# VatsalSy/gerris-fft-particles

Measured on AMD Instinct MI355X. Metric: Mcell-steps/s (projection+advection), 3D 256^3 uniform, higher is better.
Workload: dtype f64; 1 GPU; 3-D periodic Taylor-Green, 256^3 per GPU, default projection/advection parameters (SURVEY 8d config C); relax_mode=exact, parallelism=1 box, rccl_world_size=0

## Files before the change

### gerris-fft-particles_amd/csrc/gfship_internal.hpp

```cpp
#pragma once

#include <hip/hip_runtime.h>
#include <cstdio>
#include <cstdarg>
#include <cstring>
#include <vector>
#include <deque>
#include <string>
#include "gfship.h"

namespace gfship {

struct Layout {
  int n = 0;
  int px = 0;
  int xo = 1;
  int rows = 0;
  int dim = 3;
  long sy = 0;
  long sz = 0;
  size_t total = 0;
  __host__ __device__ inline long idx (int i, int j, int k) const {
    return xo + i + sy*j + sz*k;
  }
// ... 126 lines not shown
    if (e_ != hipSuccess) return gfship::hip_fail (e_, #call, __FILE__, __LINE__); } while (0)

inline hipError_t stream_wait_spin (hipStream_t st)
{
  hipError_t e;
  while ((e = hipStreamQuery (st)) == hipErrorNotReady)
    ;
  return e;
}

#define GFSHIP_CHECK(cond, code, ...) do { if (!(cond)) { \
    gfship::set_error (__VA_ARGS__); return (code); } } while (0)

Field * get_field (gfship_domain * dom, gfship_field f);
int coarse_flush (gfship_domain * dom, Field * F, int level, bool leaf_write = false);
inline long ncells (const Layout & L) {
  return L.dim == 3 ? (long) L.n*L.n*L.n : (long) L.n*L.n;
}

int launch_bc (gfship_domain * dom, Field * v, Field * v1, int level, int homogeneous);
int call_exchange (gfship_domain * dom, double * ptr, int level, int kind);
int bc_mpi_begin (gfship_domain * dom, Field * v1, int level);
int bc_mpi_end (gfship_domain * dom, Field * v, Field * v1, int level, int homogeneous);
int call_reduce (gfship_domain * dom, double * vals, int n, int op);
int call_reduce_norm (gfship_domain * dom, double * sums, int nsum, double * mx);
int comm_exchange (gfship_domain * dom, double * a, int level, int kind);
int comm_exchange_raw (gfship_domain * dom, double * const send[6], double * const recv[6], size_t count);
int comm_migrate (gfship_domain * dom, int rs, const int nsend[6], const double * const send[6],
		  int nrecv[6], std::vector<double> recv[6]);
int comm_allgather (gfship_domain * dom, const double * send, double * recv, size_t count);
// ... 27 lines not shown
int launch_residual (gfship_domain * dom, int level, const double * u, const double * rhs,
		     const double * dia, double * res);
int launch_residual_weighted (gfship_domain * dom, int level, const double * u, const double * rhs,
			      const double * dia, double * res);
int launch_poisson_weights (gfship_domain * dom, double * const alpha[3]);
RelaxOp weighted_op (gfship_domain * dom, int level);
int launch_restrict (gfship_domain * dom, unsigned dimension, int level_coarse, double * v_coarse,
		     const double * v_fine);
int launch_prolongate (gfship_domain * dom, int level_coarse, const double * v_coarse,
		       double * v_fine);
int launch_correct (gfship_domain * dom, int level, double * u, const double * dp);
int launch_fill (gfship_domain * dom, int level, double * a, double value);
int launch_residual_norm (gfship_domain * dom, int level, const double * u, const double * rhs,
			  const double * dia, double * res, double scale, double weight,
			  double * out , bool dia_zero = false);
int launch_norm_async (gfship_domain * dom, int level, const double * a, double scale, double weight);
int launch_norm (gfship_domain * dom, int level, const double * a, double scale, double weight,
		 double out[5] );

int launch_face_interp_un (gfship_domain * dom, double * const u[3], double * const un[3]);
int launch_divergence (gfship_domain * dom, double * const un[3], double * div, double dt);
int launch_correct_un (gfship_domain * dom, const double * p, double * const un[3], double dt);
int launch_centered_gradient (gfship_domain * dom, const double * p, double * const g[3]);
int launch_correct_centered (gfship_domain * dom, double * const u[3], double * const g[3], double dt);
int launch_correct_centered_coarse (gfship_domain * dom, double * const u[3], double * const g[3],
				    double dt, double * const uc[3]);
int launch_coarse_init_from (gfship_domain * dom, Field * const * v, int nf, int top);
int launch_coarse_init_levels (gfship_domain * dom, Field * const * v, int nf, int top, int bottom);
int launch_advected_face_values (gfship_domain * dom, const double * v, double * const u[3],
				 double * const un[3], double dt, int use_centered, int gradient,
				 double * const fv[6], int cmask, double visc = 0., double gsrc = 0.);
// ... 43 lines not shown
		     const double * dia, bool dia_zero, unsigned nrelax, int reps,
		     double * ms_per_loop, int * fused, double * ms_inclusive = nullptr);
int  skew_check_error (gfship_domain * dom);
int  skew_arm_ahead (gfship_domain * dom, int level, unsigned nrelax);
int  patch_resident_per_cu ();
bool prolongation_fused (gfship_domain * dom, unsigned dimension, int level, unsigned nrelax);
bool prolongation_fusable (gfship_domain * dom, unsigned dimension, int level, unsigned nrelax);
inline bool patch_level (const gfship_domain * dom, int level) { return dom->patch && !dom->weighted && dom->lay[level].n >= dom->patch_min_n; }
int  patch_pack (gfship_domain * dom, int level, SkewPlan * S, const double * u, const double * rhs,
		 const double * dia, const double * coarse = nullptr);
int  patch_unpack (gfship_domain * dom, int level, SkewPlan * S, double * u, double * add_into);
int  patch_restrict_pack (gfship_domain * dom, int level, SkewPlan * S, const double * res,
			  double * res_coarse, SkewPlan * Sc, unsigned dimension);
int  launch_restrict_pack (gfship_domain * dom, unsigned dimension, int level, Field * res,
			   bool coarse_fused);
void skew_dump_stats (gfship_domain * dom, int level);
int  skew_time_sweeps (gfship_domain * dom, int level, Field * u, const double * rhs,
		       const double * dia, bool dia_zero, int reps, double * ms_per_sweep);

}
```

### gerris-fft-particles_amd/csrc/poisson.hip

```cpp
#include "gfship_internal.hpp"
#include <cmath>
#include <cfloat>
#include <cstdlib>

using namespace gfship;

namespace gfship {

static bool weighted_pipelinable (gfship_domain * dom, unsigned dimension, int level)
{
  return dom->relax_mode == GFSHIP_RELAX_EXACT && dimension == 3 && dom->dim == 3 &&
    skew_supported (dom, level) && !dom->force_hyperplane;
}

static bool weighted_pipelined (gfship_domain * dom, unsigned dimension, int level)
{
  static const bool off = getenv ("GFSHIP_WEIGHTED_HYPERPLANES") != nullptr;
  return !off && weighted_pipelinable (dom, dimension, level);
}

static int relax_level (gfship_domain * dom, unsigned dimension, int level, double omega,
			Field * u, Field * rhs, Field * dia)
{
  u->zero[level] = false;
// ... 282 lines not shown
  if (n.w > 0.) {
    n.bias /= n.w;
    n.first /= n.w;
    n.second = sqrt (n.second/n.w);
  }
  else
    n.infty = 0.;
  *out = n;
  return GFSHIP_OK;
}

}

static int poisson_cycle (gfship_domain * dom, gfship_multilevel_params * p,
			  gfship_field u, gfship_field rhs, gfship_field dia, gfship_field res,
			  double dt, gfship_norm * norm)
{
  GFSHIP_CHECK (dom && p, GFSHIP_EINVAL, "null argument");
  GFSHIP_CHECK (p->dimension == 2 || p->dimension == 3, GFSHIP_EINVAL, "dimension must be 2 or 3");
  GFSHIP_CHECK (p->nrelax > 0 && p->erelax > 0, GFSHIP_EINVAL, "nrelax and erelax must be non zero");
  GFSHIP_CHECK (dom->unit_weights, GFSHIP_EINVAL, "call gfship_poisson_coefficients first");
  if (dom->dp_cache < 0)
    dom->dp_cache = gfship_field_alloc (dom, -1);
  gfship_field dpf = dom->dp_cache;
  if (dpf < 0) return dpf;
  Field * U = get_field (dom, u), * R = get_field (dom, rhs), * D = get_field (dom, dia),
    * S = get_field (dom, res), * DP = get_field (dom, dpf);
  int r = GFSHIP_OK;
  bool corrected = false;
  if (!U || !R || !D || !S) return GFSHIP_EINVAL;
  const int L = dom->depth;
// ... 9 lines not shown
    {
      unsigned nr = p->nrelax;
      for (int l = L; l >= 0; l--) {
	nrl[l] = nr;
	if (l > (int) minlevel) nr *= p->erelax;
      }
    }
    for (int l = 0; l <= L; l++)
      DP->zero[l] = false;
    const int ctop = dom->weighted ? -1 : coarse_cycle_top (dom, (int) minlevel);
    const int ltop = ctop >= 0 ? -1 : lattice_cycle_top (dom, (int) minlevel, D);
    for (int l = L - 1; l >= (ctop >= 0 ? ctop + 1 : ltop >= 0 ? ltop : 0); l--) {
      if (dom->relax_mode == GFSHIP_RELAX_EXACT && p->dimension == 3 && !dom->weighted &&
	  !dom->force_hyperplane && skew_supported (dom, l + 1))
	TRY (skew_arm_ahead (dom, l + 1, nrl[l + 1]));
      const bool rp = !dom->skew[l + 1].rs_ready && prolongation_fused (dom, p->dimension, l + 1, nrl[l + 1]);
      if (rp) dom->kc[dom->no_fused_restriction ? GFSHIP_KC_RESTRICTION_DECLINED : GFSHIP_KC_RESTRICTION_FUSED]++;
      if (!dom->no_fused_restriction && rp)
	TRY (launch_restrict_pack (dom, p->dimension, l + 1, S,
				   l > (int) minlevel && prolongation_fused (dom, p->dimension, l, nrl[l])));
      else
	TRY (launch_restrict (dom, p->dimension, l, S->lev[l], S->lev[l + 1]));
    }
    unsigned first = minlevel;
    if (ltop >= 0) {
      TRY (launch_lattice_cycle (dom, p->dimension, p->omega, (int) minlevel, ltop, nrl, DP, U, S));
      first = ltop + 1;
    }
    else if (ctop >= 0) {
      TRY (launch_coarse_cycle (dom, p->dimension, p->omega, (int) minlevel, ctop, nrl, DP, U, S, D));
// ... 5 lines not shown
      first = minlevel + 1;
      dom->kc[GFSHIP_KC_COARSE_END_BY_LEVEL]++;
    }
    for (unsigned l = first; l <= p->depth; l++) {
      const bool fp = prolongation_fused (dom, p->dimension, (int) l, nrl[l]);
      if (fp) dom->kc[GFSHIP_KC_PROLONGATION_FUSED]++;
      else if (prolongation_fusable (dom, p->dimension, (int) l, nrl[l])) dom->kc[GFSHIP_KC_PROLONGATION_DECLINED]++;
      if (!fp)
	TRY (launch_prolongate (dom, l - 1, DP->lev[l - 1], DP->lev[l]));
      TRY (relax_loop (dom, DP, U, p->dimension, l, p->omega, S, D, nrl[l],
		       (int) l == L ? U->lev[L] : nullptr, &corrected, fp ? DP->lev[l - 1] : nullptr));
    }
  }
  if (!corrected)
    TRY (launch_correct (dom, L, U->lev[L], DP->lev[L]));
  TRY (launch_bc (dom, U, U, L, 0));
  if (norm)
    TRY (residual_and_norm (dom, dt, U, R, D, S, norm));
  else if (dom->weighted)
    TRY (launch_residual_weighted (dom, L, U->lev[L], R->lev[L], D->lev[L], S->lev[L]));
  else
    TRY (launch_residual (dom, L, U->lev[L], R->lev[L], D->lev[L], S->lev[L]));
#undef TRY
 done:
  for (int l = 0; l <= L; l++)
    dom->skew[l].rs_ready = false;
  return r;
}

extern "C" {

int gfship_poisson_cycle (gfship_domain * dom, gfship_multilevel_params * p,
			  gfship_field u, gfship_field rhs, gfship_field dia, gfship_field res)
{
  GFSHIP_CHECK (dom != nullptr, GFSHIP_EINVAL, "null domain");
  int r = before_write (dom);
  if (r) return r;
  return poisson_cycle (dom, p, u, rhs, dia, res, 1., nullptr);
}

int gfship_poisson_solve (gfship_domain * dom, gfship_multilevel_params * par,
			  gfship_field lhs, gfship_field rhs, gfship_field res,
// ... 1 lines not shown
{
  GFSHIP_CHECK (dom && par, GFSHIP_EINVAL, "null argument");
  Field * U = get_field (dom, lhs), * R = get_field (dom, rhs), * D = get_field (dom, dia),
    * S = get_field (dom, res);
  if (!U || !R || !D || !S) return GFSHIP_EINVAL;
  GFSHIP_CHECK (dom->unit_weights, GFSHIP_EINVAL, "call gfship_poisson_coefficients first");
  { int r = before_write (dom); if (r) return r; }
  int r;
  const int L = dom->depth;
  if ((r = coarse_flush (dom, U, L, true))) return r;
  unsigned minlevel = par->minlevel;
  par->depth = L;
  par->niter = 0;

  bool deferred = par->nitermin >= 1 && par->nitermax >= 1;
  if (deferred) {
    const Layout & Ly = dom->lay[L];
    double size = 1./Ly.n;
    S->zero[L] = false;
    if (dom->weighted) {
      if ((r = launch_residual_weighted (dom, L, U->lev[L], R->lev[L], D->lev[L], S->lev[L]))) return r;
      if ((r = launch_norm_async (dom, L, S->lev[L], 1.*size*size, 1.))) return r;
    }
    else if ((r = launch_residual_norm (dom, L, U->lev[L], R->lev[L], D->lev[L], S->lev[L], 1.*size*size,
					1., nullptr, D->zero[L])))
      return r;
  }
  else {
    if ((r = residual_and_norm (dom, dt, U, R, D, S, &par->residual))) return r;
    par->residual_before = par->residual;
  }

  double res_max_before = par->residual.infty;

  while (par->niter < par->nitermin ||
	 (par->residual.infty > par->tolerance && par->niter < par->nitermax)) {
    if ((r = poisson_cycle (dom, par, lhs, rhs, dia, res, dt, &par->residual))) {
      if (deferred) {
	deferred = false;
	double s0[5];
	if (hipStreamSynchronize (dom->stream) == hipSuccess) {
	  memcpy (s0, dom->h_pinned + 8, sizeof (s0));
	  if (norm_residual_finish (dom, dt, s0, &par->residual_before) == GFSHIP_OK)
	    par->residual = par->residual_before;
	}
	else
	  memset (&par->residual_before, 0, sizeof (par->residual_before)),
	    memset (&par->residual, 0, sizeof (par->residual));
      }
      break;
    }
    if (deferred) {
// ... 80 lines not shown
```

### gerris-fft-particles_amd/csrc/poisson_kernels.hip

```cpp
#include "gfship_internal.hpp"
#include "relax_skew.hpp"
#include <algorithm>
#include <cstdlib>

namespace gfship {

struct W6 { const double * p[6]; };

template <int DIM, int OP>
__device__ __forceinline__ double relax_value (const double * __restrict__ u, long c, long sy, long sz,
					       double rhs, double dia, unsigned dimension,
					       double omega, double w, double h2, const W6 * wf = nullptr)
{
  if (OP == 2) {
    double a = dia, b = 0.;
    { const double g = wf->p[0][c]; a += g; b += g*u[c + 1]; }
    { const double g = wf->p[1][c]; a += g; b += g*u[c - 1]; }
    { const double g = wf->p[2][c]; a += g; b += g*u[c + sy]; }
    { const double g = wf->p[3][c]; a += g; b += g*u[c - sy]; }
    if (DIM == 3) {
      { const double g = wf->p[4][c]; a += g; b += g*u[c + sz]; }
      { const double g = wf->p[5][c]; a += g; b += g*u[c - sz]; }
    }
    if (dimension == 2)
// ... 1515 lines not shown
int launch_norm_async (gfship_domain * dom, int level, const double * a, double scale, double weight)
{
  const Layout & L = dom->lay[level];
  long nrows = L.dim == 3 ? (long) L.n*L.n : L.n;
  int block = L.n >= 256 ? 256 : L.n >= 128 ? 128 : 64;
  int nblocks = (int) (nrows > 1024 ? 1024 : nrows);
  double * partial = dom->d_scratch;
  double * result = dom->h_pinned + 8;
  NORM_PARTIAL_LAUNCH ();
  hipLaunchKernelGGL (norm_final_kernel, dim3 (1), dim3 (256), 0, dom->stream,
		      partial, nblocks, result);
  GFSHIP_HIP (hipGetLastError ());
  return GFSHIP_OK;
}

int launch_norm (gfship_domain * dom, int level, const double * a, double scale, double weight,
		 double out[5])
{
  const Layout & L = dom->lay[level];
  long nrows = L.dim == 3 ? (long) L.n*L.n : L.n;
  int block = L.n >= 256 ? 256 : L.n >= 128 ? 128 : 64;
  int nblocks = (int) (nrows > 1024 ? 1024 : nrows);
  double * partial = dom->d_scratch;
  double * result = dom->h_pinned;
  NORM_PARTIAL_LAUNCH ();
  hipLaunchKernelGGL (norm_final_kernel, dim3 (1), dim3 (256), 0, dom->stream,
		      partial, nblocks, result);
  GFSHIP_HIP (hipGetLastError ());
  GFSHIP_HIP (stream_wait_spin (dom->stream));
  memcpy (out, dom->h_pinned, 5*sizeof (double));
// ... 112 lines not shown
  s0 = wave_sum (s0); s1 = wave_sum (s1); s2 = wave_sum (s2); s3 = wave_max (s3); s4 = wave_sum (s4);
  int w = threadIdx.x >> 6, lane = threadIdx.x & 63;
  if (lane == 0) { sh[0][w] = s0; sh[1][w] = s1; sh[2][w] = s2; sh[3][w] = s3; sh[4][w] = s4; }
  __syncthreads ();
  if (threadIdx.x == 0) {
    int nw = blockDim.x >> 6;
    double r0 = 0., r1 = 0., r2 = 0., r3 = 0., r4 = 0.;
    for (int q = 0; q < nw; q++) {
      r0 += sh[0][q]; r1 += sh[1][q]; r2 += sh[2][q]; r3 = fmax (r3, sh[3][q]); r4 += sh[4][q];
    }
    double * p = partial + 5*(size_t) blockIdx.x;
    p[0] = r0; p[1] = r1; p[2] = r2; p[3] = r3; p[4] = r4;
  }
}

int launch_residual_norm (gfship_domain * dom, int level, const double * u, const double * rhs,
			  const double * dia, double * res, double scale, double weight,
			  double * out, bool dia_zero)
{
  const Layout & L = dom->lay[level];
  if (!power_of_two (scale)) {
    int r = launch_residual (dom, level, u, rhs, dia, res);
    if (r) return r;
    return out ? launch_norm (dom, level, res, scale, weight, out) :
      launch_norm_async (dom, level, res, scale, weight);
  }
  long nrows = L.dim == 3 ? (long) L.n*L.n : L.n;
  int block = L.n >= 256 ? 256 : L.n >= 128 ? 128 : 64;
  static int rn_blocks = 0;
  if (!rn_blocks) {
// ... 192 lines not shown
```

### gerris-fft-particles_amd/csrc/relax_patch_loop.hip

```cpp
#include "relax_skew.hpp"
#include <cstdlib>
#include <vector>

#ifndef PK_D
#define PK_D 9
#endif
#ifndef PK_DH
#define PK_DH 3
#endif
#ifndef PK_KO
#define PK_KO 0
#endif
#define PK_NTHREADS 192
#define PK_SKEW 14

namespace gfship {

typedef double d2 __attribute__((ext_vector_type(2)));

__device__ __forceinline__ void patch_arm_other_set (const SkewLoopArgs & A, int tile, int tid, int nt)
{
  if (A.arm_pairs == 0) return;
  typedef unsigned long long ull2 __attribute__((ext_vector_type(2)));
  const unsigned long long W = A.arm_cum[A.ntj*A.ntj];
// ... 827 lines not shown
  }
  const double v = __longlong_as_double ((long long) bits);
  A.un[dst] = sg == 0. ? v : sg*v;
}

struct PatchPackArgs {
  Layout L;
  int ntj, RT;
  const double * src[3];
  double * dst[3];
  int narr;
  double * add;
  const double * coarse;
  double * nat;
  Layout Lc;
};

__device__ __forceinline__ double patch_prolong (const Layout & Lc, const double * __restrict__ vc,
						 int i, int j, int k)
{
  const int pi = (i + 1)/2, pj = (j + 1)/2, pk = (k + 1)/2;
  const long p = Lc.idx (pi, pj, pk);
  const double pv = vc[p];
  double h[3];
  const long off[3] = { 1, Lc.sy, Lc.sz };
#pragma unroll
  for (int cc = 0; cc < 3; cc++) {
    double g1 = vc[p + off[cc]] - 1.*pv;
    double g2 = vc[p - off[cc]] - 1.*pv;
    h[cc] = (g1 - g2)/2.;
  }
// ... 100 lines not shown
    const double bx = pv + ((I & 1) ? qx : - qx);
    d2 o01, o23;
    {
      const double by0 = bx + qy, by1 = bx + (- qy);
      o01.x = by0 + qz;     o01.y = by1 + qz;
      o23.x = by0 + (- qz); o23.y = by1 + (- qz);
    }
    double * const row = dst + (long) rho*SK_NL;
    *(d2 *) row = o01;
    *(d2 *) (row + 128) = o23;
    if (__builtin_expect (I == 0 || I == n - 1 || side_j[0] || side_j[1] || side_k[0] || side_k[1], 0)) {
      const bool ends = I == 0 || I == n - 1;
      const double vv[4] = { o01.x, o01.y, o23.x, o23.y };
#pragma unroll
      for (int q = 0; q < 4; q++)
	if (ends || side_j[q & 1] || side_k[q >> 1])
	  A.nat[A.L.idx (I + 1, j0 - (q & 1), k0 - (q >> 1))] = vv[q];
    }
  }
}

#ifndef PP_ROWS
#define PP_ROWS 16
#endif
#define PP_SPAN (PP_ROWS + 7)
#ifndef PPR_ROWS
#define PPR_ROWS 64
#endif
#define PPR_SPAN (PPR_ROWS + 7)
#ifndef PPU_ROWS
#define PPU_ROWS 64
#endif
// ... 8 lines not shown
  const int P = tile % A.ntj, Q = tile / A.ntj;
  const int n = A.L.n;
  const long tbase = (long) tile*(A.RT + 2*SK_FP)*SK_NL + SK_FP*SK_NL;
  const int I0 = r0 - 7 - PB;
  for (int e = tid; e < 32*PP_SPAN; e += 256) {
    const int line = e / PP_SPAN, di = e % PP_SPAN;
    const int a = line & 15, db = line >> 4;
    const int I = I0 + di;
    if (I >= 0 && I < n) {
      const int j = n - (SK_T*P + a), k = n - (SK_T*Q + 2*PB + db);
      const long nidx = A.L.idx (I + 1, j, k);
      int q0 = 0;
      if (A.coarse) {
	const double v = patch_prolong (A.Lc, A.coarse, I + 1, j, k);
	buf[0][line][di] = v;
	if (I == 0 || I == n - 1 || j == 1 || j == n || k == 1 || k == n)
	  A.nat[nidx] = v;
	q0 = 1;
      }
      for (int q = q0; q < A.narr; q++)
	buf[q][line][di] = A.src[q][nidx];
    }
  }
  __syncthreads ();
  for (int e = tid; e < PP_ROWS*32; e += 256) {
    const int row = e / 32, col = e % 32;
    const int PA = col >> 2, p = col & 3;
    const int a = 2*PA + (p & 1), db = p >> 1;
    const int rho = r0 + row;
    const int I = rho - PA - PB;
    if (I >= 0 && I < n) {
      const long sidx = tbase + (long) rho*SK_NL + 128*(p >> 1) + 2*(PA + 8*PB) + (p & 1);
// ... 53 lines not shown
      double val = 0.;
#pragma unroll
      for (int id = 0; id < 8; id++)
	val += buf[2*PA + ((id >> 1) & 1) + 16*(id >> 2)][di + (id & 1)];
      const double v = A.dimension == 2 ? val : val/2.;
      const int m = I >> 1;
      const int pj = (n - SK_T*P - 2*PA) >> 1, pk = (n - SK_T*Q - 2*PB) >> 1;
      A.cnat[A.Lc.idx (m + 1, pj, pk)] = v;
      if (A.cskew) {
	const int ca = 8*(P & 1) + PA, cb = 8*(Q & 1) + PB;
	const long ctile = (P >> 1) + (long) A.cntj*(Q >> 1);
	A.cskew[ctile*(A.cRT + 2*SK_FP)*SK_NL + SK_FP*SK_NL +
		(long) (m + (ca >> 1) + (cb >> 1))*SK_NL + 128*(cb & 1) + 2*((ca >> 1) + 8*(cb >> 1)) + (ca & 1)] = v;
      }
    }
  }
}

__global__ void __launch_bounds__(256)
patch_unpack_kernel (PatchPackArgs A)
{
  __shared__ double buf[32][PPU_SPAN + 1];
  const int tid = threadIdx.x;
  const int tile = blockIdx.z, PB = blockIdx.y, r0 = blockIdx.x*PPU_ROWS;
  const int P = tile % A.ntj, Q = tile / A.ntj;
  const int n = A.L.n;
  const long tbase = (long) tile*(A.RT + 2*SK_FP)*SK_NL + SK_FP*SK_NL;
  const int I0 = r0 - 7 - PB;
  for (int e = tid; e < PPU_ROWS*32; e += 256) {
    const int row = e / 32, col = e % 32;
// ... 1 lines not shown
    const int a = 2*PA + (p & 1), db = p >> 1;
    const int rho = r0 + row;
    const int I = rho - PA - PB;
    if (I >= 0 && I < n)
      buf[a + 16*db][I - I0] = A.src[0][tbase + (long) rho*SK_NL + 128*(p >> 1) + 2*(PA + 8*PB) + (p & 1)];
  }
  __syncthreads ();
  for (int e = tid; e < 32*PPU_SPAN; e += 256) {
    const int line = e / PPU_SPAN, di = e % PPU_SPAN;
    const int a = line & 15, db = line >> 4;
    const int I = I0 + di;
    const int rho = I + (a >> 1) + PB;
    if (I >= 0 && I < n && rho >= r0 && rho < r0 + PPU_ROWS) {
      const int j = n - (SK_T*P + a), k = n - (SK_T*Q + 2*PB + db);
      const long c = A.L.idx (I + 1, j, k);
      if (A.add)
	A.add[c] += buf[line][di];
      else
	A.dst[0][c] = buf[line][di];
    }
  }
}

static bool patch_regs ()
{
  return getenv ("GFSHIP_PATCH_REGS") != nullptr;
}

int patch_resident_per_cu ()
{
  int per_cu = 0;
  hipError_t e = patch_regs () ?
    hipOccupancyMaxActiveBlocksPerMultiprocessor (&per_cu, relax_patch_loop_kernel<true>, PK_NTHREADS, 0) :
    hipOccupancyMaxActiveBlocksPerMultiprocessor (&per_cu, relax_ring_loop_kernel<true, 0>, RK_NTHREADS, 0);
  int per_cu1 = 0;
  if (e == hipSuccess)
    e = hipOccupancyMaxActiveBlocksPerMultiprocessor (&per_cu1, relax_ring_loop_kernel<true, 1>, RK_NTHREADS, 0);
  if (per_cu1 < per_cu) per_cu = per_cu1;
  return e == hipSuccess ? per_cu : 0;
}

int patch_pack (gfship_domain * dom, int level, SkewPlan * S, const double * u, const double * rhs,
		const double * dia, const double * coarse)
{
  PatchPackArgs A;
  A.add = nullptr;
  A.coarse = coarse;
  A.nat = const_cast<double *> (u);
  A.Lc = dom->lay[level > 0 ? level - 1 : 0];
  A.L = dom->lay[level]; A.ntj = S->ntj; A.RT = S->RT;
  A.narr = 0;
  A.src[A.narr] = u;   A.dst[A.narr++] = S->us;
  if (rhs) { A.src[A.narr] = rhs; A.dst[A.narr++] = S->rs; }
  if (dia) { A.src[A.narr] = dia; A.dst[A.narr++] = S->ds; }
  const int rows = A.L.n + PK_SKEW + 1;
  const bool old_pack = coarse && getenv ("GFSHIP_OLD_PROLONG_PACK");
  if (coarse) dom->kc[old_pack ? GFSHIP_KC_PROLONG_PACK_OLD : GFSHIP_KC_PROLONG_PACK_NEW]++;
  if (coarse && !old_pack) {
    PatchPackArgs Pr = A;
    Pr.narr = 1;
    dim3 pgrid ((rows + PR_ROWS*PR_WAVES - 1)/(PR_ROWS*PR_WAVES), S->ntj*S->ntj);
    hipLaunchKernelGGL (patch_prolong_kernel, pgrid, dim3 (64*PR_WAVES), 0, dom->stream, Pr);
// ... 16 lines not shown
  PatchRestrictArgs A;
  A.L = dom->lay[level]; A.Lc = dom->lay[level - 1];
  A.ntj = S->ntj; A.RT = S->RT;
  A.src = res; A.dst = S->rs;
  A.cnat = res_coarse;
  A.cskew = Sc ? Sc->rs : nullptr;
  A.cntj = Sc ? Sc->ntj : 0; A.cRT = Sc ? Sc->RT : 0;
  A.dimension = dimension;
  const int rows = A.L.n + PK_SKEW + 1;
  dim3 grid ((rows + PPR_ROWS - 1)/PPR_ROWS, 8, S->ntj*S->ntj);
  hipLaunchKernelGGL (patch_restrict_pack_kernel, grid, dim3 (256), 0, dom->stream, A);
  GFSHIP_HIP (hipGetLastError ());
  return GFSHIP_OK;
}

int patch_unpack (gfship_domain * dom, int level, SkewPlan * S, double * u, double * add_into)
{
  PatchPackArgs A;
  A.coarse = nullptr; A.nat = nullptr; A.Lc = dom->lay[level];
  A.L = dom->lay[level]; A.ntj = S->ntj; A.RT = S->RT;
  A.narr = 1;
  A.src[0] = S->us; A.dst[0] = u; A.add = add_into;
  const int rows = A.L.n + PK_SKEW + 1;
  dim3 grid ((rows + PPU_ROWS - 1)/PPU_ROWS, 8, S->ntj*S->ntj);
  hipLaunchKernelGGL (patch_unpack_kernel, grid, dim3 (256), 0, dom->stream, A);
  GFSHIP_HIP (hipGetLastError ());
  return GFSHIP_OK;
}

int patch_loop_launch (gfship_domain * dom, const SkewLoopArgs & A, int ntiles, bool has_dia,
		       unsigned nrelax, float * ms)
{
  if (ms) GFSHIP_HIP (hipEventRecord (dom->ev0, dom->stream));
  if (A.op == 1)
    hipLaunchKernelGGL ((relax_ring_loop_kernel<true, 1>), dim3 (ntiles), dim3 (RK_NTHREADS), 0, dom->stream, A);
  else if (patch_regs ()) {
    if (has_dia)
// ... 26 lines not shown
```

### gerris-fft-particles_amd/csrc/relax_skew.hip

```cpp
#include "relax_skew.hpp"
#include <cstdlib>

namespace gfship {

template <bool HAS_DIA>
__global__ void __launch_bounds__(SK_NL)
relax_skew_kernel (SkewArgs A)
{
  constexpr int XS = SK_T + 1;
  __shared__ double X[2][XS*XS];
  __shared__ double Y[2][XS*XS];
  __shared__ unsigned s_tile;

  const int tid = threadIdx.x;
  const int a = tid & (SK_T - 1), b = tid >> 4;
  const int n = A.L.n;
  const int ntj = A.ntj;
  const long tstride = (long) (A.RT + 2*SK_FP)*SK_NL;
  const long hstride = (long) SK_HROWS (n)*SK_T;

  if (tid == 0)
    s_tile = A.order[atomicAdd (A.ticket, 1u)];
  __syncthreads ();
  const int tile = s_tile;
// ... 450 lines not shown
  SkewPlan * S;
  int r;
  if ((r = skew_plan (dom, level, &S))) return r;
  double * u = dp->lev[level];
  if ((r = skew_loop_trial (dom, level, S, nrelax, bc))) return r;
  if (op && op->kind == 2) {
    if ((r = skew_pack_weights (dom, level, S, op))) return r;
    dia_zero = false;
  }
  const bool fusedp = prolong_from != nullptr && bc && patch_level (dom, level);
  const double * rhs_pack = S->rs_ready && patch_level (dom, level) ? nullptr : rhs;
  S->rs_ready = false;
  if (prolong_from && !fusedp)
    if ((r = launch_prolongate (dom, level - 1, prolong_from, u))) return r;
  if (fusedp && (r = skew_pack (dom, level, S, u, rhs_pack, dia_zero ? nullptr : dia, prolong_from))) return r;
  if (bc && (r = launch_bc (dom, ubc, dp, level, 1))) return r;
  if (!fusedp && (r = skew_pack (dom, level, S, u, rhs_pack, dia_zero ? nullptr : dia))) return r;
  if (!dom->no_fused_loop && skew_loop_supported (dom, level, nrelax, bc)) {
    if ((r = skew_loop_run (dom, level, S, u, !dia_zero, nrelax, nullptr, ubc, op))) return r;
    return skew_unpack (dom, level, S, u, correct_into);
  }
  for (unsigned q = 0; q < nrelax; q++) {
    if ((r = skew_sweep (dom, level, S, u, !dia_zero, op))) return r;
    if (bc && q + 1 < nrelax && (r = launch_bc (dom, ubc, dp, level, 1))) return r;
  }
  return skew_unpack (dom, level, S, u, correct_into);
}

int launch_restrict_pack (gfship_domain * dom, unsigned dimension, int level, Field * res, bool coarse_fused)
{
  SkewPlan * S, * Sc = nullptr;
  int r;
  if ((r = skew_plan (dom, level, &S))) return r;
  if ((r = skew_loop_trial (dom, level, S, 4, true))) return r;
  if (coarse_fused) {
    if ((r = skew_plan (dom, level - 1, &Sc))) return r;
    if ((r = skew_loop_trial (dom, level - 1, Sc, 4, true))) return r;
  }
  res->zero[level - 1] = false;
  if ((r = patch_restrict_pack (dom, level, S, res->lev[level], res->lev[level - 1], Sc, dimension))) return r;
  S->rs_ready = true;
  if (Sc) Sc->rs_ready = true;
  return GFSHIP_OK;
}

void skew_dump_stats (gfship_domain * dom, int level)
{
  SkewPlan & S = dom->skew[level];
  if (!S.stats) return;
  (void) hipStreamSynchronize (dom->stream);
  int nt = S.ntj*S.ntj;
  std::vector<u64> h (4*nt);
  (void) hipMemcpy (h.data (), S.stats, h.size ()*sizeof (u64), hipMemcpyDeviceToHost);
  u64 t0 = ~0ull;
  for (int q = 0; q < nt; q++) if (h[4*q] < t0) t0 = h[4*q];
  for (int Q = 0; Q < S.ntj; Q++)
    for (int P = 0; P < S.ntj; P++) {
      int q = P + S.ntj*Q;
// ... 139 lines not shown
```

### gerris-fft-particles_amd/gfship/__init__.py

```python
import ctypes as C
import os
import sys

import numpy as np

_PKG = os.path.dirname(os.path.dirname(os.path.abspath(__file__)))
LIB_PATH = os.environ.get("GFSHIP_LIB", os.path.join(_PKG, "lib", "libgfship.so"))

SIDE_PERIODIC, SIDE_BOUNDARY, SIDE_EXTERNAL = 0, 1, 2
BC_SYMMETRY, BC_DIRICHLET, BC_NEUMANN = 0, 1, 2
RELAX_EXACT, RELAX_REDBLACK, RELAX_EXACT_HYPERPLANE, RELAX_EXACT_PER_SWEEP = 0, 1, 2, 3


class GfshipError(RuntimeError):
    pass


class Norm(C.Structure):
    _fields_ = [("bias", C.c_double), ("first", C.c_double), ("second", C.c_double),
                ("infty", C.c_double), ("w", C.c_double)]


class MultilevelParams(C.Structure):
    _fields_ = [("tolerance", C.c_double), ("nrelax", C.c_uint), ("erelax", C.c_uint),
# ... 159 lines not shown

UNIQUE_ID_BYTES = 128

KERNEL_COUNT_NAMES = (
    "PREDICT_SWEEP", "PREDICT_SWEEP_MPI", "PREDICT_TILED", "PREDICT_TILED_MPI", "PREDICT_GENERAL",
    "ADVECT3_SWEEP2", "ADVECT3_SWEEP2_MPI", "ADVECT3_SWEEP1", "ADVECT3_TILED", "ADVECT3_TILED_MPI",
    "ADVECT1_TILED_VELOCITY", "ADVECT1_TILED_TRACER", "ADVECT_GENERAL", "CORRECTION_FUSED",
    "CORRECTION_DECLINED", "DIVERGENCE_FUSED", "DIVERGENCE_DECLINED", "DIVERGENCE_SEPARATE",
    "PROJECT_PAIRS", "PROJECT_SCALAR", "RESIDUAL_PAIRS", "RESIDUAL_SCALAR", "RN_BLOCKS_LIMIT",
    "RN_BLOCKS_MAX", "ROWS2D", "HYPERPLANES_2D", "DIFFUSION_PIPELINED", "DIFFUSION_HYPERPLANES",
    "WEIGHTED_PIPELINED", "WEIGHTED_HYPERPLANES", "PROLONGATION_FUSED", "PROLONGATION_DECLINED",
    "RESTRICTION_FUSED", "RESTRICTION_DECLINED", "PROLONG_PACK_NEW", "PROLONG_PACK_OLD",
    "ARM_AHEAD", "ARM_AHEAD_DECLINED", "ARM_INLINE", "PATCH_LOOP_KERNEL_ARMS",
    "PATCH_LOOP_HOST_ARMS", "XCD_SCOPE_ON", "XCD_SCOPE_OFF", "XCD_NEAR_MODE", "XCD_PLACE_ON",
    "XCD_PLACE_OFF", "COARSE_CYCLES", "COARSE_THREADS", "COARSE_END_BY_LEVEL",
)
KERNEL_COUNT_VALUES = ("RN_BLOCKS_LIMIT", "RN_BLOCKS_MAX", "XCD_NEAR_MODE", "COARSE_THREADS")


def comm_available():
    _check(lib().gfship_comm_available())


def comm_unique_id():
    buf = C.create_string_buffer(UNIQUE_ID_BYTES)
    _check(lib().gfship_comm_unique_id(buf))
    return buf.raw


def lib():
# ... 631 lines not shown
```

### include/gfship.h

```cpp
#ifndef GFSHIP_H
#define GFSHIP_H

#include <stddef.h>

#ifdef __cplusplus
extern "C" {
#endif

#define GFSHIP_VERSION   1
#define GFSHIP_MAXLEVEL  12

enum { GFSHIP_OK = 0, GFSHIP_EINVAL = -1, GFSHIP_ENODEVICE = -2, GFSHIP_ENOMEM = -3,
       GFSHIP_EHIP = -4, GFSHIP_EUNSUPPORTED = -5 };

enum { GFSHIP_SIDE_PERIODIC = 0,
       GFSHIP_SIDE_BOUNDARY = 1,
       GFSHIP_SIDE_EXTERNAL = 2 };

enum { GFSHIP_BC_SYMMETRY = 0, GFSHIP_BC_DIRICHLET = 1, GFSHIP_BC_NEUMANN = 2 };

enum { GFSHIP_RELAX_EXACT = 0, GFSHIP_RELAX_REDBLACK = 1, GFSHIP_RELAX_EXACT_HYPERPLANE = 2,
       GFSHIP_RELAX_EXACT_PER_SWEEP = 3 };

typedef struct gfship_domain gfship_domain;
// ... 229 lines not shown
  GFSHIP_KC_PROLONG_PACK_NEW,
  GFSHIP_KC_PROLONG_PACK_OLD,
  GFSHIP_KC_ARM_AHEAD,
  GFSHIP_KC_ARM_AHEAD_DECLINED,
  GFSHIP_KC_ARM_INLINE,
  GFSHIP_KC_PATCH_LOOP_KERNEL_ARMS,
  GFSHIP_KC_PATCH_LOOP_HOST_ARMS,
  GFSHIP_KC_XCD_SCOPE_ON,
  GFSHIP_KC_XCD_SCOPE_OFF,
  GFSHIP_KC_XCD_NEAR_MODE,
  GFSHIP_KC_XCD_PLACE_ON,
  GFSHIP_KC_XCD_PLACE_OFF,
  GFSHIP_KC_COARSE_CYCLES,
  GFSHIP_KC_COARSE_THREADS,
  GFSHIP_KC_COARSE_END_BY_LEVEL,
  GFSHIP_KC_COUNT
};
int  gfship_domain_kernel_counts (gfship_domain * dom, unsigned long long * counts, int n);
#define GFSHIP_UNIQUE_ID_BYTES 128
int  gfship_comm_available (void);
int  gfship_comm_unique_id (void * id);
int  gfship_domain_comm_init (gfship_domain * dom, const void * unique_id, int rank, int nranks,
			      const int lattice[3]);
int  gfship_domain_comm_size (gfship_domain * dom);
int  gfship_domain_comm_stats (gfship_domain * dom, unsigned long long * messages,
			       unsigned long long * bytes);
int  gfship_domain_comm_destroy (gfship_domain * dom);

int  gfship_halo_pack (gfship_domain * dom, const void * dev_ptr, int level, int side, void * dev_buf);
int  gfship_halo_unpack (gfship_domain * dom, void * dev_ptr, int level, int side, const void * dev_buf);
// ... 65 lines not shown
```

Before: 2766 Mcell-steps/s.

## Fuse initial residual, norm and restriction; write periodic ghosts from producers

Adds a kernel that computes the leaf-level initial residual, accumulates the residual norm partials, and writes both the skewed residual pack and the restricted coarse residual in one pass. The first multigrid cycle then skips its own leaf restriction. For fully periodic domains, the prolongation-pack and unpack kernels now write periodic ghost images directly, so separate boundary-condition launches after the fused prolong and final correction are skipped. This cuts kernel launches and full-grid passes, at the cost of extra scattered ghost stores and more specialized code paths with many eligibility conditions.

```diff
diff --git a/gerris-fft-particles_amd/csrc/gfship_internal.hpp b/gerris-fft-particles_amd/csrc/gfship_internal.hpp
--- a/gerris-fft-particles_amd/csrc/gfship_internal.hpp
+++ b/gerris-fft-particles_amd/csrc/gfship_internal.hpp
@@ -164,6 +164,11 @@
 
 Field * get_field (gfship_domain * dom, gfship_field f);
 int coarse_flush (gfship_domain * dom, Field * F, int level, bool leaf_write = false);
+inline bool all_periodic (const gfship_domain * dom) {
+  for (int d = 0; d < 6; d++)
+    if (dom->side[d] != GFSHIP_SIDE_PERIODIC) return false;
+  return dom->dim == 3 && !dom->has_external;
+}
 inline long ncells (const Layout & L) {
   return L.dim == 3 ? (long) L.n*L.n*L.n : (long) L.n*L.n;
 }
@@ -221,7 +226,9 @@
 int launch_residual_norm (gfship_domain * dom, int level, const double * u, const double * rhs,
 			  const double * dia, double * res, double scale, double weight,
 			  double * out , bool dia_zero = false);
+bool residual_pairs ();
 int launch_norm_async (gfship_domain * dom, int level, const double * a, double scale, double weight);
+int launch_norm_final_async (gfship_domain * dom, int nblocks);
 int launch_norm (gfship_domain * dom, int level, const double * a, double scale, double weight,
 		 double out[5] );
 
@@ -295,6 +302,12 @@
 			  double * res_coarse, SkewPlan * Sc, unsigned dimension);
 int  launch_restrict_pack (gfship_domain * dom, unsigned dimension, int level, Field * res,
 			   bool coarse_fused);
+int  patch_residual_restrict_pack (gfship_domain * dom, int level, SkewPlan * S, const double * u,
+				   const double * rhs, const double * dia, double * res_coarse, SkewPlan * Sc,
+				   unsigned dimension, double scale, double weight, int * nblocks_out);
+int  launch_residual_restrict_pack (gfship_domain * dom, unsigned dimension, int level, const double * u,
+				    const double * rhs, const double * dia, Field * res, bool coarse_fused,
+				    double scale, double weight);
 void skew_dump_stats (gfship_domain * dom, int level);
 int  skew_time_sweeps (gfship_domain * dom, int level, Field * u, const double * rhs,
 		       const double * dia, bool dia_zero, int reps, double * ms_per_sweep);
diff --git a/gerris-fft-particles_amd/csrc/poisson.hip b/gerris-fft-particles_amd/csrc/poisson.hip
--- a/gerris-fft-particles_amd/csrc/poisson.hip
+++ b/gerris-fft-particles_amd/csrc/poisson.hip
@@ -320,7 +320,7 @@
 
 static int poisson_cycle (gfship_domain * dom, gfship_multilevel_params * p,
 			  gfship_field u, gfship_field rhs, gfship_field dia, gfship_field res,
-			  double dt, gfship_norm * norm)
+			  double dt, gfship_norm * norm, bool leaf_restricted = false)
 {
   GFSHIP_CHECK (dom && p, GFSHIP_EINVAL, "null argument");
   GFSHIP_CHECK (p->dimension == 2 || p->dimension == 3, GFSHIP_EINVAL, "dimension must be 2 or 3");
@@ -360,6 +360,8 @@
       if (dom->relax_mode == GFSHIP_RELAX_EXACT && p->dimension == 3 && !dom->weighted &&
 	  !dom->force_hyperplane && skew_supported (dom, l + 1))
 	TRY (skew_arm_ahead (dom, l + 1, nrl[l + 1]));
+      if (leaf_restricted && l == L - 1)
+	continue;
       const bool rp = !dom->skew[l + 1].rs_ready && prolongation_fused (dom, p->dimension, l + 1, nrl[l + 1]);
       if (rp) dom->kc[dom->no_fused_restriction ? GFSHIP_KC_RESTRICTION_DECLINED : GFSHIP_KC_RESTRICTION_FUSED]++;
       if (!dom->no_fused_restriction && rp)
@@ -395,7 +397,10 @@
   }
   if (!corrected)
     TRY (launch_correct (dom, L, U->lev[L], DP->lev[L]));
-  TRY (launch_bc (dom, U, U, L, 0));
+  if (corrected && patch_level (dom, L) && all_periodic (dom))
+    dom->kc[GFSHIP_KC_BC_BY_PRODUCER]++;
+  else
+    TRY (launch_bc (dom, U, U, L, 0));
   if (norm)
     TRY (residual_and_norm (dom, dt, U, R, D, S, norm));
   else if (dom->weighted)
@@ -407,6 +412,25 @@
   for (int l = 0; l <= L; l++)
     dom->skew[l].rs_ready = false;
   return r;
+}
+
+static bool initial_residual_fused (gfship_domain * dom, const gfship_multilevel_params * par, Field * D)
+{
+  const int L = dom->depth;
+  if (L < 1 || dom->weighted || dom->has_external || dom->no_fused_restriction || !residual_pairs ())
+    return false;
+  if (par->dimension != 3 || par->nrelax == 0 || par->erelax == 0 || !dom->unit_weights)
+    return false;
+  if (dom->skew[L].rs_ready || !prolongation_fused (dom, par->dimension, L, par->nrelax))
+    return false;
+  int e;
+  const double size = 1./dom->lay[L].n;
+  if (frexp (1.*size*size, &e) != 0.5)
+    return false;
+  int minlevel = par->minlevel > (unsigned) L ? L : (int) par->minlevel;
+  const int ctop = coarse_cycle_top (dom, minlevel);
+  const int ltop = ctop >= 0 ? -1 : lattice_cycle_top (dom, minlevel, D);
+  return L - 1 >= (ctop >= 0 ? ctop + 1 : ltop >= 0 ? ltop : 0);
 }
 
 extern "C" {
@@ -438,11 +462,24 @@
   par->niter = 0;
 
   bool deferred = par->nitermin >= 1 && par->nitermax >= 1;
+  bool leaf_restricted = false;
   if (deferred) {
     const Layout & Ly = dom->lay[L];
     double size = 1./Ly.n;
     S->zero[L] = false;
-    if (dom->weighted) {
+    if (initial_residual_fused (dom, par, D)) {
+      unsigned ml = par->minlevel > (unsigned) L ? L : par->minlevel;
+      const bool coarse_fused = L - 1 > (int) ml &&
+	prolongation_fused (dom, par->dimension, L - 1, par->nrelax*(L > (int) ml ? par->erelax : 1));
+      dom->kc[GFSHIP_KC_RESTRICTION_FUSED]++;
+      dom->kc[GFSHIP_KC_RESIDUAL_RESTRICT_FUSED]++;
+      if ((r = launch_residual_restrict_pack (dom, par->dimension, L, U->lev[L], R->lev[L],
+					      D->zero[L] ? nullptr : D->lev[L], S, coarse_fused,
+					      1.*size*size, 1.)))
+	return r;
+      leaf_restricted = true;
+    }
+    else if (dom->weighted) {
       if ((r = launch_residual_weighted (dom, L, U->lev[L], R->lev[L], D->lev[L], S->lev[L]))) return r;
       if ((r = launch_norm_async (dom, L, S->lev[L], 1.*size*size, 1.))) return r;
     }
@@ -459,7 +496,9 @@
 
   while (par->niter < par->nitermin ||
 	 (par->residual.infty > par->tolerance && par->niter < par->nitermax)) {
-    if ((r = poisson_cycle (dom, par, lhs, rhs, dia, res, dt, &par->residual))) {
+    const bool restricted = leaf_restricted;
+    leaf_restricted = false;
+    if ((r = poisson_cycle (dom, par, lhs, rhs, dia, res, dt, &par->residual, restricted))) {
       if (deferred) {
 	deferred = false;
 	double s0[5];
diff --git a/gerris-fft-particles_amd/csrc/poisson_kernels.hip b/gerris-fft-particles_amd/csrc/poisson_kernels.hip
--- a/gerris-fft-particles_amd/csrc/poisson_kernels.hip
+++ b/gerris-fft-particles_amd/csrc/poisson_kernels.hip
@@ -1553,6 +1553,14 @@
   return GFSHIP_OK;
 }
 
+int launch_norm_final_async (gfship_domain * dom, int nblocks)
+{
+  hipLaunchKernelGGL (norm_final_kernel, dim3 (1), dim3 (256), 0, dom->stream,
+		      dom->d_scratch, nblocks, dom->h_pinned + 8);
+  GFSHIP_HIP (hipGetLastError ());
+  return GFSHIP_OK;
+}
+
 int launch_norm (gfship_domain * dom, int level, const double * a, double scale, double weight,
 		 double out[5])
 {
@@ -1695,6 +1703,12 @@
   }
 }
 
+bool residual_pairs ()
+{
+  static const bool pairs = getenv ("GFSHIP_RN_SCALAR") == nullptr;
+  return pairs;
+}
+
 int launch_residual_norm (gfship_domain * dom, int level, const double * u, const double * rhs,
 			  const double * dia, double * res, double scale, double weight,
 			  double * out, bool dia_zero)
diff --git a/gerris-fft-particles_amd/csrc/relax_patch_loop.hip b/gerris-fft-particles_amd/csrc/relax_patch_loop.hip
--- a/gerris-fft-particles_amd/csrc/relax_patch_loop.hip
+++ b/gerris-fft-particles_amd/csrc/relax_patch_loop.hip
@@ -865,7 +865,20 @@
   const double * coarse;
   double * nat;
   Layout Lc;
+  int periodic;
 };
+
+__device__ __forceinline__ void store_periodic_images (const Layout & L, double * __restrict__ a,
+						       int i, int j, int k, double v)
+{
+  const int n = L.n;
+  if (i == 1) a[L.idx (n + 1, j, k)] = v;
+  if (i == n) a[L.idx (0, j, k)] = v;
+  if (j == 1) a[L.idx (i, n + 1, k)] = v;
+  if (j == n) a[L.idx (i, 0, k)] = v;
+  if (k == 1) a[L.idx (i, j, n + 1)] = v;
+  if (k == n) a[L.idx (i, j, 0)] = v;
+}
 
 __device__ __forceinline__ double patch_prolong (const Layout & Lc, const double * __restrict__ vc,
 						 int i, int j, int k)
@@ -996,8 +1009,11 @@
       const double vv[4] = { o01.x, o01.y, o23.x, o23.y };
 #pragma unroll
       for (int q = 0; q < 4; q++)
-	if (ends || side_j[q & 1] || side_k[q >> 1])
+	if (ends || side_j[q & 1] || side_k[q >> 1]) {
 	  A.nat[A.L.idx (I + 1, j0 - (q & 1), k0 - (q >> 1))] = vv[q];
+	  if (A.periodic)
+	    store_periodic_images (A.L, A.nat, I + 1, j0 - (q & 1), k0 - (q >> 1), vv[q]);
+	}
     }
   }
 }
@@ -1036,8 +1052,11 @@
       if (A.coarse) {
 	const double v = patch_prolong (A.Lc, A.coarse, I + 1, j, k);
 	buf[0][line][di] = v;
-	if (I == 0 || I == n - 1 || j == 1 || j == n || k == 1 || k == n)
+	if (I == 0 || I == n - 1 || j == 1 || j == n || k == 1 || k == n) {
 	  A.nat[nidx] = v;
+	  if (A.periodic)
+	    store_periodic_images (A.L, A.nat, I + 1, j, k, v);
+	}
 	q0 = 1;
       }
       for (int q = q0; q < A.narr; q++)
@@ -1121,6 +1140,140 @@
 		(long) (m + (ca >> 1) + (cb >> 1))*SK_NL + 128*(cb & 1) + 2*((ca >> 1) + 8*(cb >> 1)) + (ca & 1)] = v;
       }
     }
+  }
+}
+
+#define RRP_PAIRS (PPR_ROWS/2 + 1)
+
+struct PatchResidualArgs {
+  PatchRestrictArgs R;
+  const double * u, * rhs, * dia;
+  double inv, weight;
+  double * partial;
+  int nchunks;
+  int total;
+};
+
+__global__ void __launch_bounds__(256)
+patch_residual_restrict_pack_kernel (PatchResidualArgs B)
+{
+  const PatchRestrictArgs & A = B.R;
+  __shared__ double buf[32][PPR_SPAN + 2];
+  __shared__ double sh[5][4];
+  const int tid = threadIdx.x;
+  const int n = A.L.n;
+  const long sy = A.L.sy, sz = A.L.sz;
+  const double * __restrict__ const u = B.u;
+  const double * __restrict__ const rhs = B.rhs;
+  const double * __restrict__ const dia = B.dia;
+  const double inv = B.inv, weight = B.weight;
+  double s0 = 0., s1 = 0., s2 = 0., s3 = 0., s4 = 0.;
+  for (int item = blockIdx.x; item < B.total; item += gridDim.x) {
+    const int r0 = (item % B.nchunks)*PPR_ROWS, PB = (item / B.nchunks) & 7, tile = item / (8*B.nchunks);
+    const int P = tile % A.ntj, Q = tile / A.ntj;
+    const long tbase = (long) tile*(A.RT + 2*SK_FP)*SK_NL + SK_FP*SK_NL;
+    const int I0 = r0 - 7 - PB;
+    for (int e = tid; e < 32*RRP_PAIRS; e += 256) {
+      const int line = e / RRP_PAIRS, pr = e % RRP_PAIRS;
+      const int la = line & 15, db = line >> 4, PA = la >> 1;
+      const int I = ((r0 - PA - PB) & ~1) + 2*pr;
+      if (I < 0 || I >= n) continue;
+      const int j = n - (SK_T*P + la), k = n - (SK_T*Q + 2*PB + db);
+      const long c = A.L.idx (I + 1, j, k);
+      const d2 uc = *(const d2 *) (u + c);
+      const double ul = u[c - 1], ur = u[c + 2];
+      const d2 ut = *(const d2 *) (u + c + sy), ub = *(const d2 *) (u + c - sy);
+      const d2 uf = *(const d2 *) (u + c + sz), uk = *(const d2 *) (u + c - sz);
+      const d2 rh = *(const d2 *) (rhs + c);
+      d2 di = { 0., 0. };
+      if (dia) di = *(const d2 *) (dia + c);
+      d2 out;
+      {
+	double a = di.x, b = 0.;
+	a += 1.; b += 1.*uc.y;
+	a += 1.; b += 1.*ul;
+	a += 1.; b += 1.*ut.x;
+	a += 1.; b += 1.*ub.x;
+	a += 1.; b += 1.*uf.x;
+	a += 1.; b += 1.*uk.x;
+	out.x = rh.x - (b - uc.x*a);
+      }
+      {
+	double a = di.y, b = 0.;
+	a += 1.; b += 1.*ur;
+	a += 1.; b += 1.*uc.x;
+	a += 1.; b += 1.*ut.y;
+	a += 1.; b += 1.*ub.y;
+	a += 1.; b += 1.*uf.y;
+	a += 1.; b += 1.*uk.y;
+	out.y = rh.y - (b - uc.y*a);
+      }
+#pragma unroll
+      for (int q = 0; q < 2; q++) {
+	const double raw = q ? out.y : out.x;
+	const int row = I + q + PA + PB - r0;
+	if (row >= 0 && row <= PPR_ROWS)
+	  buf[line][I + q - I0] = raw;
+	if (row >= 0 && row < PPR_ROWS) {
+	  double val = raw*inv;
+	  s0 += weight*val;
+	  val = fabs (val);
+	  s3 = fmax (s3, val);
+	  s1 += weight*val;
+	  s2 += weight*val*val;
+	  s4 += raw;
+	}
+      }
+    }
+    __syncthreads ();
+    for (int e = tid; e < PPR_ROWS*32; e += 256) {
+      const int row = e / 32, col = e % 32;
+      const int PA = col >> 2, p = col & 3;
+      const int a = 2*PA + (p & 1), db = p >> 1;
+      const int rho = r0 + row;
+      const int I = rho - PA - PB;
+      if (I >= 0 && I < n)
+	A.dst[tbase + (long) rho*SK_NL + 128*(p >> 1) + 2*(PA + 8*PB) + (p & 1)] = buf[a + 16*db][I - I0];
+    }
+    for (int e = tid; e < 8*(PPR_ROWS/2); e += 256) {
+      const int PA = e / (PPR_ROWS/2), mi = e % (PPR_ROWS/2);
+      const int par = (PA + PB + r0) & 1;
+      const int row = 2*mi + par;
+      const int I = r0 + row - PA - PB;
+      if (I >= 0 && I < n) {
+	const int di = I - I0;
+	double val = 0.;
+#pragma unroll
+	for (int id = 0; id < 8; id++)
+	  val += buf[2*PA + ((id >> 1) & 1) + 16*(id >> 2)][di + (id & 1)];
+	const double v = A.dimension == 2 ? val : val/2.;
+	const int m = I >> 1;
+	const int pj = (n - SK_T*P - 2*PA) >> 1, pk = (n - SK_T*Q - 2*PB) >> 1;
+	A.cnat[A.Lc.idx (m + 1, pj, pk)] = v;
+	if (A.cskew) {
+	  const int ca = 8*(P & 1) + PA, cb = 8*(Q & 1) + PB;
+	  const long ctile = (P >> 1) + (long) A.cntj*(Q >> 1);
+	  A.cskew[ctile*(A.cRT + 2*SK_FP)*SK_NL + SK_FP*SK_NL +
+		  (long) (m + (ca >> 1) + (cb >> 1))*SK_NL + 128*(cb & 1) + 2*((ca >> 1) + 8*(cb >> 1)) + (ca & 1)] = v;
+	}
+      }
+    }
+    __syncthreads ();
+  }
+  for (int o = 32; o > 0; o >>= 1) {
+    s0 += __shfl_down (s0, o, 64); s1 += __shfl_down (s1, o, 64); s2 += __shfl_down (s2, o, 64);
+    s3 = fmax (s3, __shfl_down (s3, o, 64)); s4 += __shfl_down (s4, o, 64);
+  }
+  const int wv = tid >> 6;
+  if ((tid & 63) == 0) { sh[0][wv] = s0; sh[1][wv] = s1; sh[2][wv] = s2; sh[3][wv] = s3; sh[4][wv] = s4; }
+  __syncthreads ();
+  if (tid == 0) {
+    double r0 = 0., r1 = 0., r2 = 0., r3 = 0., r4 = 0.;
+    for (int q = 0; q < 4; q++) {
+      r0 += sh[0][q]; r1 += sh[1][q]; r2 += sh[2][q]; r3 = fmax (r3, sh[3][q]); r4 += sh[4][q];
+    }
+    double * p = B.partial + 5*(size_t) blockIdx.x;
+    p[0] = r0; p[1] = r1; p[2] = r2; p[3] = r3; p[4] = r4;
   }
 }
 
@@ -1152,8 +1305,12 @@
     if (I >= 0 && I < n && rho >= r0 && rho < r0 + PPU_ROWS) {
       const int j = n - (SK_T*P + a), k = n - (SK_T*Q + 2*PB + db);
       const long c = A.L.idx (I + 1, j, k);
-      if (A.add)
-	A.add[c] += buf[line][di];
+      if (A.add) {
+	const double v = A.add[c] + buf[line][di];
+	A.add[c] = v;
+	if (A.periodic && (I == 0 || I == n - 1 || j == 1 || j == n || k == 1 || k == n))
+	  store_periodic_images (A.L, A.add, I + 1, j, k, v);
+      }
       else
 	A.dst[0][c] = buf[line][di];
     }
@@ -1184,6 +1341,7 @@
   PatchPackArgs A;
   A.add = nullptr;
   A.coarse = coarse;
+  A.periodic = coarse && all_periodic (dom);
   A.nat = const_cast<double *> (u);
   A.Lc = dom->lay[level > 0 ? level - 1 : 0];
   A.L = dom->lay[level]; A.ntj = S->ntj; A.RT = S->RT;
@@ -1230,6 +1388,34 @@
   return GFSHIP_OK;
 }
 
+#define RRP_MAX_GROUPS 8192
+int patch_residual_restrict_pack (gfship_domain * dom, int level, SkewPlan * S, const double * u,
+				  const double * rhs, const double * dia, double * res_coarse, SkewPlan * Sc,
+				  unsigned dimension, double scale, double weight, int * nblocks_out)
+{
+  PatchResidualArgs B;
+  PatchRestrictArgs & A = B.R;
+  A.L = dom->lay[level]; A.Lc = dom->lay[level - 1];
+  A.ntj = S->ntj; A.RT = S->RT;
+  A.src = nullptr; A.dst = S->rs;
+  A.cnat = res_coarse;
+  A.cskew = Sc ? Sc->rs : nullptr;
+  A.cntj = Sc ? Sc->ntj : 0; A.cRT = Sc ? Sc->RT : 0;
+  A.dimension = dimension;
+  B.u = u; B.rhs = rhs; B.dia = dia;
+  B.inv = 1./scale; B.weight = weight;
+  B.partial = dom->d_scratch;
+  const int rows = A.L.n + PK_SKEW + 1;
+  B.nchunks = (rows + PPR_ROWS - 1)/PPR_ROWS;
+  B.total = B.nchunks*8*S->ntj*S->ntj;
+  const int nblocks = B.total < RRP_MAX_GROUPS ? B.total : RRP_MAX_GROUPS;
+  GFSHIP_CHECK ((size_t) 5*nblocks <= dom->scratch_doubles, GFSHIP_EINVAL, "reduction scratch too small");
+  hipLaunchKernelGGL (patch_residual_restrict_pack_kernel, dim3 (nblocks), dim3 (256), 0, dom->stream, B);
+  GFSHIP_HIP (hipGetLastError ());
+  *nblocks_out = nblocks;
+  return GFSHIP_OK;
+}
+
 int patch_unpack (gfship_domain * dom, int level, SkewPlan * S, double * u, double * add_into)
 {
   PatchPackArgs A;
@@ -1237,6 +1423,7 @@
   A.L = dom->lay[level]; A.ntj = S->ntj; A.RT = S->RT;
   A.narr = 1;
   A.src[0] = S->us; A.dst[0] = u; A.add = add_into;
+  A.periodic = add_into && all_periodic (dom);
   const int rows = A.L.n + PK_SKEW + 1;
   dim3 grid ((rows + PPU_ROWS - 1)/PPU_ROWS, 8, S->ntj*S->ntj);
   hipLaunchKernelGGL (patch_unpack_kernel, grid, dim3 (256), 0, dom->stream, A);
diff --git a/gerris-fft-particles_amd/csrc/relax_skew.hip b/gerris-fft-particles_amd/csrc/relax_skew.hip
--- a/gerris-fft-particles_amd/csrc/relax_skew.hip
+++ b/gerris-fft-particles_amd/csrc/relax_skew.hip
@@ -488,7 +488,9 @@
   if (prolong_from && !fusedp)
     if ((r = launch_prolongate (dom, level - 1, prolong_from, u))) return r;
   if (fusedp && (r = skew_pack (dom, level, S, u, rhs_pack, dia_zero ? nullptr : dia, prolong_from))) return r;
-  if (bc && (r = launch_bc (dom, ubc, dp, level, 1))) return r;
+  if (bc && fusedp && all_periodic (dom))
+    dom->kc[GFSHIP_KC_BC_BY_PRODUCER]++;
+  else if (bc && (r = launch_bc (dom, ubc, dp, level, 1))) return r;
   if (!fusedp && (r = skew_pack (dom, level, S, u, rhs_pack, dia_zero ? nullptr : dia))) return r;
   if (!dom->no_fused_loop && skew_loop_supported (dom, level, nrelax, bc)) {
     if ((r = skew_loop_run (dom, level, S, u, !dia_zero, nrelax, nullptr, ubc, op))) return r;
@@ -516,6 +518,27 @@
   S->rs_ready = true;
   if (Sc) Sc->rs_ready = true;
   return GFSHIP_OK;
+}
+
+int launch_residual_restrict_pack (gfship_domain * dom, unsigned dimension, int level, const double * u,
+				   const double * rhs, const double * dia, Field * res, bool coarse_fused,
+				   double scale, double weight)
+{
+  SkewPlan * S, * Sc = nullptr;
+  int r, nblocks = 0;
+  if ((r = skew_plan (dom, level, &S))) return r;
+  if ((r = skew_loop_trial (dom, level, S, 4, true))) return r;
+  if (coarse_fused) {
+    if ((r = skew_plan (dom, level - 1, &Sc))) return r;
+    if ((r = skew_loop_trial (dom, level - 1, Sc, 4, true))) return r;
+  }
+  res->zero[level] = res->zero[level - 1] = false;
+  if ((r = patch_residual_restrict_pack (dom, level, S, u, rhs, dia, res->lev[level - 1], Sc, dimension,
+					 scale, weight, &nblocks)))
+    return r;
+  S->rs_ready = true;
+  if (Sc) Sc->rs_ready = true;
+  return launch_norm_final_async (dom, nblocks);
 }
 
 void skew_dump_stats (gfship_domain * dom, int level)
diff --git a/gerris-fft-particles_amd/gfship/__init__.py b/gerris-fft-particles_amd/gfship/__init__.py
--- a/gerris-fft-particles_amd/gfship/__init__.py
+++ b/gerris-fft-particles_amd/gfship/__init__.py
@@ -197,6 +197,7 @@
     "ARM_AHEAD", "ARM_AHEAD_DECLINED", "ARM_INLINE", "PATCH_LOOP_KERNEL_ARMS",
     "PATCH_LOOP_HOST_ARMS", "XCD_SCOPE_ON", "XCD_SCOPE_OFF", "XCD_NEAR_MODE", "XCD_PLACE_ON",
     "XCD_PLACE_OFF", "COARSE_CYCLES", "COARSE_THREADS", "COARSE_END_BY_LEVEL",
+    "RESIDUAL_RESTRICT_FUSED", "BC_BY_PRODUCER",
 )
 KERNEL_COUNT_VALUES = ("RN_BLOCKS_LIMIT", "RN_BLOCKS_MAX", "XCD_NEAR_MODE", "COARSE_THREADS")
 
diff --git a/include/gfship.h b/include/gfship.h
--- a/include/gfship.h
+++ b/include/gfship.h
@@ -267,6 +267,8 @@
   GFSHIP_KC_COARSE_CYCLES,
   GFSHIP_KC_COARSE_THREADS,
   GFSHIP_KC_COARSE_END_BY_LEVEL,
+  GFSHIP_KC_RESIDUAL_RESTRICT_FUSED,
+  GFSHIP_KC_BC_BY_PRODUCER,
   GFSHIP_KC_COUNT
 };
 int  gfship_domain_kernel_counts (gfship_domain * dom, unsigned long long * counts, int n);
```

After: 2765 Mcell-steps/s, median of 2. No clear change (-0.1%).
